# tsolomko/SWCompression

Measured on AMD Instinct MI355X. Metric: decompressed GiB/s, higher is better.
Workload: dtype u8; 1 GPU; 100000 x 64 KiB gzip members (BASELINE configs[1]; 4096 distinct, tiled at distinct addresses); codec=deflate, units_per_gpu=100000, unit_bytes=65536, compressed_bytes_per_gpu=2122936095, decompressed_bytes_per_gpu=6553600000, parallelism=1 x independent shards (weak scaling)

## Files before the change

__graft_entry__.py:

```python
import os
import subprocess
import sys

ROOT = os.path.dirname(os.path.abspath(__file__))
if ROOT not in sys.path:
    sys.path.insert(0, ROOT)


def build():
    from swcompression_amd import build as _b
    _b.build(force=True)
    import swcompression_amd
    from swcompression_amd import _lib
    _lib.load()
    subprocess.run(["make", "-s", "-C", os.path.join(ROOT, "oracle")], check=True)
    sys.path.insert(0, os.path.join(ROOT, "tests"))
    import _emu
    _emu.build(force=True)
    import _emu_bgzf
    _emu_bgzf.build(force=True)


def smoke():
    import torch
    assert torch.cuda.is_available(), "smoke() needs the MI355X"
    sys.path.insert(0, os.path.join(ROOT, "tests"))
    import _oracle as O
    import swcompression_amd as swc
    from swcompression_amd import corpus
    from swcompression_amd.batch import DeviceBatch
    assert swc.device_available(), "libswc_hip.so found no gfx950 device"
    plains = [corpus.p_text(65536, 900 + i) for i in range(96)] + [corpus.p_mix(20000, 5), b"", corpus.p_rand(3000, 1)]
    units = [corpus.deflate_raw(p) for p in plains]
    b = DeviceBatch("deflate", units, [max(len(p), 1) for p in plains], device="cuda:0")
    from swcompression_amd import _lib
    lib = _lib.load()
    expected = [O.deflate(u) for u in units]
    b.launch(sync=True)
    r = b.results()
    for i, (p, (st, out, cons)) in enumerate(zip(plains, expected)):
        assert (st, out) == (0, p)
        assert int(r["status"][i]) == 0 and int(r["out_len"][i]) == len(p) and int(r["in_consumed"][i]) == cons
        assert b.output(i, len(p)) == p, "HIP output differs from the oracle on unit %d" % i
# ... 9 lines not shown
```

include/swc_hip.h:

```cpp
#ifndef SWC_HIP_H
#define SWC_HIP_H

#include <stddef.h>
#include <stdint.h>
#include "swc_status.h"

#ifdef __cplusplus
extern "C" {
#endif

typedef enum swc_codec {
    SWC_CODEC_DEFLATE = 1,
    SWC_CODEC_LZ4_BLOCK = 2,
    SWC_CODEC_LZMA2 = 3,
    SWC_CODEC_LZMA = 4,
    SWC_CODEC_BZIP2_BLOCK = 5,
    SWC_CODEC_DELTA = 6,
    SWC_CODEC_LZ4_COMPRESS = 7,
    SWC_CODEC_DEFLATE_COMPRESS = 8,
    SWC_CODEC_DEFLATE_COMPRESS_DYNAMIC = 9
} swc_codec;

typedef struct swc_job {
    const uint8_t* in;
// ... 2 lines not shown
    uint64_t out_cap;
    uint64_t out_len;
    uint64_t in_consumed;
    int32_t status;
    int32_t aux;
    const uint8_t* dict;
    uint64_t dict_len;
} swc_job;

typedef struct swc_batch_opts {
    int32_t device;
    void* stream;
    int32_t synchronize;
    int32_t reserved;
} swc_batch_opts;

int swc_batch_decompress(int codec, swc_job* jobs, size_t n, const swc_batch_opts* opts);

size_t swc_batch_workspace_bytes(int codec, size_t n_jobs, uint64_t max_out_cap);
int swc_batch_decompress_ws(int codec, swc_job* jobs, size_t n, void* workspace, size_t workspace_bytes,
                            const swc_batch_opts* opts);

int swc_batch_crc32(const swc_job* jobs, size_t n, uint32_t* crcs, const swc_batch_opts* opts);

typedef enum swc_checksum {
    SWC_SUM_CRC32 = 1,
    SWC_SUM_ADLER32 = 2,
    SWC_SUM_CRC64 = 3,
    SWC_SUM_BZIP2_CRC32 = 4,
    SWC_SUM_XXH32 = 5
} swc_checksum;
int swc_batch_checksum(int kind, const swc_job* jobs, size_t n, uint64_t* sums, const swc_batch_opts* opts);

int swc_deflate_decompress(const uint8_t* in, size_t in_len, uint8_t** out, size_t* out_len, size_t* in_consumed);

int swc_bzip2_decompress(const uint8_t* in, size_t in_len, uint8_t** out, size_t* out_len, size_t* in_consumed);
int swc_bzip2_multi_decompress(const uint8_t* in, size_t in_len, uint8_t** out, size_t* out_len, size_t** sizes, size_t* n_streams);

int swc_lzma_decompress(const uint8_t* in, size_t in_len, int lc, int lp, int pb, int64_t dict_size,
                        int64_t uncompressed_size, uint8_t** out, size_t* out_len, size_t* in_consumed);
int swc_lzma_alone_decompress(const uint8_t* in, size_t in_len, uint8_t** out, size_t* out_len);
int swc_lzma2_decompress(const uint8_t* in, size_t in_len, uint8_t dict_byte, uint8_t** out, size_t* out_len, size_t* in_consumed);
int swc_lzma2_decompress_data(const uint8_t* in, size_t in_len, uint8_t** out, size_t* out_len);

int swc_lz4_decompress(const uint8_t* in, size_t in_len, const uint8_t* dict, size_t dict_len, int64_t dict_id,
                       uint8_t** out, size_t* out_len, size_t* in_consumed);
// ... 106 lines not shown
```

swcompression_amd/_lib.py:

```python
import ctypes as C
import os

_HERE = os.path.dirname(os.path.abspath(__file__))
LIB_PATH = os.environ.get("SWC_LIB") or os.path.join(_HERE, "libswc_hip.so")


class SwcJob(C.Structure):
    _fields_ = [("in_", C.c_void_p), ("in_len", C.c_uint64), ("out", C.c_void_p), ("out_cap", C.c_uint64),
                ("out_len", C.c_uint64), ("in_consumed", C.c_uint64), ("status", C.c_int32), ("aux", C.c_int32),
                ("dict", C.c_void_p), ("dict_len", C.c_uint64)]


class SwcGzipExtraField(C.Structure):
    _fields_ = [("si1", C.c_uint8), ("si2", C.c_uint8), ("bytes", C.c_void_p), ("len", C.c_size_t)]


class SwcBatchOpts(C.Structure):
    _fields_ = [("device", C.c_int32), ("stream", C.c_void_p), ("synchronize", C.c_int32), ("reserved", C.c_int32)]


_lib = None


def load():
# ... 11 lines not shown
        raise ImportError("libswc_hip.so is missing and could not be built: the MI355X engine is required")
    lib = C.CDLL(LIB_PATH)
    u8pp = C.POINTER(C.POINTER(C.c_uint8))
    szp = C.POINTER(C.c_size_t)
    szpp = C.POINTER(szp)
    I = C.c_int

    def sig(name, res, *args):
        f = getattr(lib, name)
        f.restype = res
        f.argtypes = list(args)

    sig("swc_free", None, C.c_void_p)
    sig("swc_trim", I)
    sig("swc_device_available", I)
    sig("swc_version", C.c_char_p)
    sig("swc_set_tuning", I, C.c_char_p, I)
    sig("swc_last_phase_ms", I, C.POINTER(C.c_float), I)
    sig("swc_batch_decompress", I, I, C.c_void_p, C.c_size_t, C.POINTER(SwcBatchOpts))
    sig("swc_batch_crc32", I, C.c_void_p, C.c_size_t, C.c_void_p, C.POINTER(SwcBatchOpts))
    sig("swc_batch_checksum", I, I, C.c_void_p, C.c_size_t, C.c_void_p, C.POINTER(SwcBatchOpts))
    sig("swc_batch_workspace_bytes", C.c_size_t, I, C.c_size_t, C.c_uint64)
    sig("swc_batch_decompress_ws", I, I, C.c_void_p, C.c_size_t, C.c_void_p, C.c_size_t, C.POINTER(SwcBatchOpts))
    for n in ("swc_deflate_decompress", "swc_bzip2_decompress"):
        sig(n, I, C.c_char_p, C.c_size_t, u8pp, szp, szp)
    for n in ("swc_gzip_unarchive", "swc_zlib_unarchive", "swc_xz_unarchive", "swc_lzma_alone_decompress", "swc_lzma2_decompress_data"):
        sig(n, I, C.c_char_p, C.c_size_t, u8pp, szp)
    for n in ("swc_gzip_multi_unarchive", "swc_xz_split_unarchive", "swc_bzip2_multi_decompress"):
        sig(n, I, C.c_char_p, C.c_size_t, u8pp, szp, szpp, szp)
    sig("swc_lzma_decompress", I, C.c_char_p, C.c_size_t, I, I, I, C.c_int64, C.c_int64, u8pp, szp, szp)
    sig("swc_lzma2_decompress", I, C.c_char_p, C.c_size_t, C.c_uint8, u8pp, szp, szp)
    sig("swc_lz4_decompress", I, C.c_char_p, C.c_size_t, C.c_char_p, C.c_size_t, C.c_int64, u8pp, szp, szp)
    sig("swc_lz4_multi_decompress", I, C.c_char_p, C.c_size_t, C.c_char_p, C.c_size_t, C.c_int64, u8pp, szp, szpp, szp)
    sig("swc_deflate_compress", I, C.c_char_p, C.c_size_t, u8pp, szp)
    sig("swc_bzip2_compress", I, C.c_char_p, C.c_size_t, I, u8pp, szp)
    sig("swc_zlib_archive", I, C.c_char_p, C.c_size_t, u8pp, szp)
    sig("swc_deflate_compress_dynamic", I, C.c_char_p, C.c_size_t, u8pp, szp)
    sig("swc_zlib_archive_dynamic", I, C.c_char_p, C.c_size_t, u8pp, szp)
    for n in ("swc_gzip_archive", "swc_gzip_archive_dynamic"):
        sig(n, I, C.c_char_p, C.c_size_t, C.c_char_p, C.c_size_t, C.c_char_p, C.c_size_t, I, I, I, I, C.c_int64,
            C.c_void_p, C.c_size_t, u8pp, szp)
    sig("swc_bgzf_bound", C.c_size_t, C.c_size_t, C.c_size_t)
    sig("swc_bgzf_workspace_bytes", C.c_size_t, C.c_size_t, C.c_size_t)
    sig("swc_batch_bgzf_archive", I, C.c_void_p, C.c_uint64, C.c_uint64, I, C.c_void_p, C.c_uint64, C.c_void_p, C.c_void_p,
        C.c_void_p, C.c_size_t, C.POINTER(SwcBatchOpts))
    sig("swc_bgzf_archive", I, C.c_char_p, C.c_size_t, C.c_size_t, I, u8pp, szp, szpp, szp)
# ... 22 lines not shown
```

swcompression_amd/batch.py:

```python
import ctypes as C

import numpy as np

from . import _lib

CODECS = {"deflate": 1, "lz4_block": 2, "lzma2": 3, "lzma": 4, "bzip2_block": 5, "delta": 6, "lz4_compress": 7, "deflate_compress": 8,
          "deflate_compress_dynamic": 9}

JOB_DTYPE = np.dtype([("in", "<u8"), ("in_len", "<u8"), ("out", "<u8"), ("out_cap", "<u8"), ("out_len", "<u8"),
                      ("in_consumed", "<u8"), ("status", "<i4"), ("aux", "<i4"), ("dict", "<u8"), ("dict_len", "<u8")])
assert JOB_DTYPE.itemsize == C.sizeof(_lib.SwcJob) == 72


def _align(x, a=16):
    return (x + a - 1) // a * a


class DeviceBatch:

    def __init__(self, codec, units, caps, aux=None, extra=None, dict_values=None, tile=1, device="cuda:0", replicate_inputs=True,
                 select=None):
        import torch
        self.torch = torch
        self.lib = _lib.load()
# ... 31 lines not shown
        self.d_out = torch.empty(out_total + 16, dtype=torch.uint8, device=self.device)
        jobs = np.zeros(self.n, dtype=JOB_DTYPE)
        jobs["in"] = self.d_in.data_ptr() + ((t_idx - np.uint64(t0)) * np.uint64(in_round) if replicate_inputs else 0) + in_off[k_idx]
        jobs["in_len"] = lens[k_idx]
        jobs["out"] = self.d_out.data_ptr() + out_off
        jobs["out_cap"] = caps[k_idx]
        jobs["status"] = 902
        if aux is not None:
            jobs["aux"] = np.array(aux, dtype=np.int32)[k_idx]
        if extra is not None:
            jobs["dict_len"] = np.array(extra, dtype=np.uint64)[k_idx]
        if dict_values is not None:
            jobs["dict"] = np.array(dict_values, dtype=np.uint64)[k_idx]
        self._out_off = out_off.astype(np.int64)
        self.unit_index = k_idx
        self.caps = caps[k_idx]
        self.in_lens = lens[k_idx]
        self._jobs_host = jobs
        self.d_jobs = torch.from_numpy(jobs.view(np.uint8).copy()).to(self.device)
        ws = self.lib.swc_batch_workspace_bytes(self.codec, self.n, int(caps.max()) if nd else 0)
        self.d_ws = torch.empty(max(ws, 16), dtype=torch.uint8, device=self.device)
        self.ws_bytes = ws
        self._crc_buf = None
        torch.cuda.synchronize(self.device)

    @property
    def total_in(self):
        return int(self.in_lens.sum())

    def launch(self, sync=False):
        torch = self.torch
        opts = _lib.SwcBatchOpts(self.device.index if self.device.index is not None else -1,
                                 torch.cuda.current_stream(self.device).cuda_stream, 1 if sync else 0, 0)
        st = self.lib.swc_batch_decompress_ws(self.codec, self.d_jobs.data_ptr(), self.n, self.d_ws.data_ptr(),
                                              self.ws_bytes, C.byref(opts))
        if st:
            raise RuntimeError("swc_batch_decompress failed with status %d" % st)

    def crc32(self):
        torch = self.torch
        d = torch.empty(self.n, dtype=torch.int32, device=self.device)
        opts = _lib.SwcBatchOpts(self.device.index if self.device.index is not None else -1,
                                 torch.cuda.current_stream(self.device).cuda_stream, 1, 0)
        st = self.lib.swc_batch_crc32(self.d_jobs.data_ptr(), self.n, d.data_ptr(), C.byref(opts))
        if st:
            raise RuntimeError("swc_batch_crc32 failed with status %d" % st)
        return d.cpu().numpy().view(np.uint32)

    def crc32_async(self):
        torch = self.torch
        if self._crc_buf is None:
            self._crc_buf = torch.empty(self.n, dtype=torch.int32, device=self.device)
        opts = _lib.SwcBatchOpts(self.device.index if self.device.index is not None else -1,
                                 torch.cuda.current_stream(self.device).cuda_stream, 0, 0)
        st = self.lib.swc_batch_crc32(self.d_jobs.data_ptr(), self.n, self._crc_buf.data_ptr(), C.byref(opts))
        if st:
            raise RuntimeError("swc_batch_crc32 failed with status %d" % st)

    CHECKSUMS = {"crc32": 1, "adler32": 2, "crc64": 3, "bzip2crc32": 4, "xxh32": 5}

    def checksum(self, kind):
        torch = self.torch
        d = torch.empty(self.n, dtype=torch.int64, device=self.device)
        opts = _lib.SwcBatchOpts(self.device.index if self.device.index is not None else -1,
                                 torch.cuda.current_stream(self.device).cuda_stream, 1, 0)
        st = self.lib.swc_batch_checksum(self.CHECKSUMS[kind], self.d_jobs.data_ptr(), self.n, d.data_ptr(), C.byref(opts))
        if st:
            raise RuntimeError("swc_batch_checksum failed with status %d" % st)
        return d.cpu().numpy().view(np.uint64)

    def wipe_results(self):
        self.d_out.zero_()
        jobs = self._jobs_host.copy()
        jobs["status"] = 902
        jobs["out_len"] = 0
        jobs["in_consumed"] = 0
        self.d_jobs.copy_(self.torch.from_numpy(jobs.view(np.uint8)).to(self.device))
        if self._crc_buf is not None:
            self._crc_buf.zero_()

    def results(self):
        self.torch.cuda.synchronize(self.device)
        return self.d_jobs.cpu().numpy().view(JOB_DTYPE)

    def output(self, i, n=None):
        r = self.results() if n is None else None
        ln = int(min(r["out_len"][i], r["out_cap"][i])) if n is None else n
        o = int(self._out_off[i])
        return self.d_out[o:o + ln].cpu().numpy().tobytes()


def bgzf_workspace_bytes(n_bytes, block_size=65280):
    return _lib.load().swc_bgzf_workspace_bytes(int(n_bytes), int(block_size))

# ... 18 lines not shown
```

swcompression_amd/csrc/api.cpp:

```cpp
#include <algorithm>
#include <atomic>
#include <map>
#include <chrono>
#include <functional>
#include <stdio.h>
#include <stdlib.h>
#include <mutex>
#include <thread>
#include <system_error>
#include <vector>
#include <string.h>
#include "host_util.h"
#include "launch.h"
#include "framing.h"

static_assert(sizeof(swc_job) == sizeof(swc::Job), "swc_job and swc::Job must have the same layout");
static_assert(offsetof(swc_job, status) == offsetof(swc::Job, status), "layout");
static_assert(offsetof(swc_job, dict_len) == offsetof(swc::Job, dict_len), "layout");

namespace swc {

static size_t env_mib(const char* name, size_t dflt) {
    const char* v = getenv(name);
    if (!v || !*v) return dflt;
// ... 268 lines not shown
        uint8_t* up = pinned_stage(0, up_bytes);
        if (!up) { up_fallback.resize(up_bytes); up = up_fallback.data(); }
        for (const Staged& st : staged) if (st.len) memcpy(up + st.off, st.p, st.len);
        Job* jobs = reinterpret_cast<Job*>(up + in_bytes);
        for (size_t k = 0; k < m; k++) {
            const HostUnit& u = units[pending[k]];
            if (u.dict && u.dict_len) memcpy(up + dict_off[k], u.dict, u.dict_len);
            Job& j = jobs[k];
            j.in = d_in + in_off[k];
            j.in_len = u.in_len;
            j.out = d_out + out_off[k];
            j.out_cap = cap[pending[k]];
            j.out_len = 0;
            j.in_consumed = 0;
            j.status = SWC_E_DEVICE;
            j.aux = u.aux;
            j.dict = u.dict ? d_in + dict_off[k] : reinterpret_cast<const uint8_t*>((uintptr_t)u.dict_value);
            j.dict_len = u.dict ? u.dict_len : u.extra;
        }
        if (!ws_off.empty()) memcpy(up + in_bytes + jobs_bytes, ws_off.data(), ws_off.size() * sizeof(uint64_t));
        tr.mark("stage inputs (pinned)", up_bytes);
        if (hipMemcpyAsync(d_in, up, up_bytes, hipMemcpyHostToDevice, stream) != hipSuccess) return SWC_E_DEVICE;
        const uint64_t* d_off = !ws_off.empty() ? reinterpret_cast<const uint64_t*>(d_jobs + jobs_bytes) : nullptr;
        if (launch_codec(codec, reinterpret_cast<Job*>(d_jobs), m, d_ws.ptr(), ws_bytes, stream, d_off) != hipSuccess) return SWC_E_DEVICE;
        if (sum_kind && launch_checksum(sum_kind, reinterpret_cast<const Job*>(d_jobs), m, reinterpret_cast<uint64_t*>(d_sums), stream) != hipSuccess) return SWC_E_DEVICE;
        stat_add(0, 1);
        stat_add(1, (long long)m);
        std::vector<uint8_t> down_fallback;
        uint8_t* down = pinned_stage(1, down_bytes);
        if (!down) { down_fallback.resize(down_bytes); down = down_fallback.data(); }
        if (hipMemcpyAsync(down, d_jobs, down_bytes, hipMemcpyDeviceToHost, stream) != hipSuccess) return SWC_E_DEVICE;
        tr.mark("issue launch + copies");
        if (hipStreamSynchronize(stream) != hipSuccess) return SWC_E_DEVICE;
        tr.mark("H2D + kernels + D2H", down_bytes);
        const Job* res = reinterpret_cast<const Job*>(down);
        const uint64_t* sums = reinterpret_cast<const uint64_t*>(down + jobs_bytes + off_bytes);
        const uint8_t* outs = down + jobs_bytes + off_bytes + sum_bytes;

        std::vector<size_t> next;
        std::vector<CopyOut> done;
        done.reserve(m);
        for (size_t k = 0; k < m; k++) {
            HostUnit& u = units[pending[k]];
            const Job& j = res[k];
            if (j.status == SWC_E_NEED_WORKSPACE && !want_ws) {
                next.push_back(pending[k]);
                continue;
            }
            if (j.status == SWC_E_NEED_WORKSPACE && per_job_ws && ws_extra[pending[k]] == 0) {
                ws_extra[pending[k]] = ((u.in_len * 16 + ((size_t)64 << 10)) + 15) & ~(size_t)15;
                next.push_back(pending[k]);
                continue;
            }
            if (j.status == SWC_E_NEED_WORKSPACE && codec == SWC_CODEC_BZIP2_BLOCK && cap[pending[k]] < ((size_t)15 << 20)) {
                cap[pending[k]] = std::min<size_t>(cap[pending[k]] * 4, (size_t)15 << 20);
                next.push_back(pending[k]);
                continue;
            }
            const size_t grow_limit = codec == SWC_CODEC_BZIP2_BLOCK ? (size_t)1 << 30 : (size_t)1 << 34;
            if (j.status == SWC_E_CAPACITY && !u.cap_exact && cap[pending[k]] < grow_limit) {
                size_t want = j.out_len > cap[pending[k]] ? (size_t)j.out_len : cap[pending[k]] * 4;
                cap[pending[k]] = want;
                next.push_back(pending[k]);
                continue;
            }
            u.status = (j.status == SWC_E_NEED_WORKSPACE && codec == SWC_CODEC_BZIP2_BLOCK) ? (int)SWC_E_CAPACITY : j.status;
            u.aux_out = j.aux;
            u.in_consumed = (size_t)j.in_consumed;
            const size_t produced = (size_t)std::min<uint64_t>(j.out_len, j.out_cap);
            u.out_size = produced;
            u.in_dst = u.dst != nullptr && produced <= u.dst_cap;
            if (sum_kind && u.sum_kind == sum_kind) { u.sum = sums[k]; u.sum_valid = true; }
            done.push_back(CopyOut{&u, outs + out_off[k], produced});
        }
        copy_out(done);
        tr.mark("copy out", out_total);
        if (!next.empty() && !want_ws)
            for (size_t k = 0; k < m; k++)
                if (res[k].status == SWC_E_NEED_WORKSPACE) { want_ws = true; break; }
        next.insert(next.end(), deferred.begin(), deferred.end());
        pending.swap(next);
    }
    for (size_t i : pending) units[i].status = SWC_E_CAPACITY;
    return SWC_OK;
}

}

using namespace swc;

extern "C" {

int swc_set_tuning(const char* key, int value) try {
    if (!key) return SWC_E_INVALID_ARGUMENT;
    if (!strcmp(key, "phase_timing") && (value == 0 || value == 1)) { set_phase_timing(value); return SWC_OK; }
// ... 55 lines not shown
void swc_free(void* p) { host_result_free(p); }

size_t swc_batch_workspace_bytes(int codec, size_t n_jobs, uint64_t max_out_cap) {
    (void)max_out_cap;
    switch (codec) {
        case SWC_CODEC_LZMA:
        case SWC_CODEC_LZMA2: return n_jobs * lzma_spill_bytes_per_job();
        case SWC_CODEC_BZIP2_BLOCK: return n_jobs * bzip2_ws_bytes_per_job((size_t)max_out_cap + 64);
        case SWC_CODEC_DEFLATE: return n_jobs * inflate_ws_bytes_per_job(max_out_cap);
        case SWC_CODEC_LZ4_BLOCK: return n_jobs * lz4_ws_bytes_per_job(max_out_cap);
        default: return 0;
    }
}

int swc_batch_decompress_ws(int codec, swc_job* jobs, size_t n, void* workspace, size_t workspace_bytes,
                            const swc_batch_opts* opts) try {
    if (!device_ready()) return SWC_E_DEVICE;
    if (n && !jobs) return SWC_E_INVALID_ARGUMENT;
    if (opts && opts->device >= 0 && hipSetDevice(opts->device) != hipSuccess) return SWC_E_DEVICE;
    hipStream_t stream = opts ? static_cast<hipStream_t>(opts->stream) : nullptr;
    hipError_t e = launch_codec(codec, reinterpret_cast<Job*>(jobs), n, workspace, workspace_bytes, stream);
    if (e == hipErrorInvalidValue) return SWC_E_INVALID_ARGUMENT;
    if (e != hipSuccess) return SWC_E_DEVICE;
    if (opts && opts->synchronize && hipStreamSynchronize(stream) != hipSuccess) return SWC_E_DEVICE;
    return SWC_OK;
} catch (...) {
    return SWC_E_DEVICE;
}

int swc_batch_crc32(const swc_job* jobs, size_t n, uint32_t* crcs, const swc_batch_opts* opts) try {
    if (!device_ready()) return SWC_E_DEVICE;
    if (n && (!jobs || !crcs)) return SWC_E_INVALID_ARGUMENT;
    if (opts && opts->device >= 0 && hipSetDevice(opts->device) != hipSuccess) return SWC_E_DEVICE;
    hipStream_t stream = opts ? static_cast<hipStream_t>(opts->stream) : nullptr;
    if (launch_crc32(reinterpret_cast<const Job*>(jobs), n, crcs, stream) != hipSuccess) return SWC_E_DEVICE;
    if (opts && opts->synchronize && hipStreamSynchronize(stream) != hipSuccess) return SWC_E_DEVICE;
    return SWC_OK;
} catch (...) {
    return SWC_E_DEVICE;
}

int swc_batch_checksum(int kind, const swc_job* jobs, size_t n, uint64_t* sums, const swc_batch_opts* opts) try {
    if (!device_ready()) return SWC_E_DEVICE;
    if (kind < SWC_SUM_CRC32 || kind > SWC_SUM_XXH32 || (n && (!jobs || !sums))) return SWC_E_INVALID_ARGUMENT;
    if (opts && opts->device >= 0 && hipSetDevice(opts->device) != hipSuccess) return SWC_E_DEVICE;
    hipStream_t stream = opts ? static_cast<hipStream_t>(opts->stream) : nullptr;
// ... 40 lines not shown
```

swcompression_amd/csrc/kernels.hip:

```cpp
#include <hip/hip_runtime.h>
#include <cstddef>
#include <mutex>
#include <atomic>
#include <vector>
#include "swc_common.h"
#include "inflate_lane.h"
#include "inflate_sync.h"
#include "lz_resolve.h"
#include "lz_copy.h"
#include "lz4_lane.h"
#include "lz4_wave.h"
#include "lz4_comp.h"
#include "deflate_comp.h"
#include "lzma_wave.h"
#include "bzip2_block.h"
#include "bzip2_team.h"
#include "crc32_group.h"
#include "crc32_wave.h"
#include "checksum_group.h"
#include "delta_group.h"
#include "bgzf_pack.h"
#include "launch.h"

namespace swc {

struct WsMap {
    uint8_t* base;
    size_t stride;
    const uint64_t* off;
    __device__ uint8_t* area(uint32_t g) const { return base ? base + (off ? (size_t)off[g] : (size_t)g * stride) : nullptr; }
    __device__ size_t bytes(uint32_t g) const { return off ? (size_t)(off[g + 1] - off[g]) : stride; }
};

__device__ __forceinline__ uint32_t xcd_job(uint32_t b, uint32_t n) {
    const uint32_t per = n >> 3;
    return b < (per << 3) ? (b & 7u) * per + (b >> 3) : b;
}

constexpr int kOrderClasses = 256;
constexpr size_t kOrderMin = 2048;
__device__ __forceinline__ uint32_t order_class(uint64_t len) {
// ... 62 lines not shown
#define SWC_SYNC_WAVES_PER_SIMD 4
#endif
static thread_local uint64_t* g_prof = nullptr;
void set_profile_buffer(void* p) { g_prof = static_cast<uint64_t*>(p); }
__global__ __launch_bounds__(64, SWC_SYNC_WAVES_PER_SIMD) void swc_inflate_sync_kernel(Job* __restrict__ jobs, uint32_t n, WsMap wm, uint64_t* prof, const uint32_t* __restrict__ order) {
    __shared__ __attribute__((aligned(16))) inflate::SyncLds sync_lds;
    uint32_t g = job_of(order, blockIdx.x, n);
    if (g >= n) return;
    Job job = jobs[g];
    inflate::inflate_sync_job(job, &sync_lds, wm.area(g), wm.bytes(g), (int)threadIdx.x, kWave, prof ? prof + 32 * (size_t)g : nullptr);
    if (threadIdx.x == 0) put_result(jobs, g, job);
}

constexpr int kInflateResolveThreads = 512, kInflateRingLog2 = 16;
constexpr uint32_t kInflateKeep = 32768;
__global__ __launch_bounds__(kInflateResolveThreads) void swc_lz_resolve_kernel(const Job* __restrict__ jobs, uint32_t n, WsMap wm, uint64_t* prof, const uint32_t* __restrict__ order) {
    __shared__ __attribute__((aligned(16))) lzr::Lds<kInflateResolveThreads, kInflateRingLog2> lzr_lds;
    uint32_t g = job_of(order, blockIdx.x, n);
    if (g >= n) return;
    Job job = jobs[g];
    lzr::resolve_job<kInflateResolveThreads, kInflateRingLog2, kInflateKeep>(job, wm.area(g), wm.bytes(g), &lzr_lds, prof ? prof + 32 * (size_t)g + 16 : nullptr);
}

template <typename CFG, int RM = 0>
__device__ __forceinline__ void lz_copy_body(const Job* __restrict__ jobs, uint32_t n, const WsMap& wm, const uint32_t* __restrict__ order) {
    __shared__ __attribute__((aligned(16))) lzc::Lds<CFG::kWin> lds;
    uint32_t g = job_of(order, blockIdx.x, n);
    if (g >= n) return;
    Job job = jobs[g];
    if (job.dict != nullptr) return;
    lzc::copy_job<CFG, RM>(job, wm.area(g), wm.bytes(g), &lds);
}
#ifndef SWC_LZC_WAVES
#define SWC_LZC_WAVES 6
#endif
#ifndef SWC_LZ4_RECORD_MODE
#define SWC_LZ4_RECORD_MODE 2
#endif
#ifndef SWC_LZC4_WAVES
#define SWC_LZC4_WAVES 5
#endif
__global__ __launch_bounds__(64) __attribute__((amdgpu_waves_per_eu(SWC_LZC_WAVES, SWC_LZC_WAVES))) void swc_lz_copy_kernel(const Job* __restrict__ jobs, uint32_t n, WsMap wm, const uint32_t* __restrict__ order) {
    lz_copy_body<lzc::CfgDeflate>(jobs, n, wm, order);
}
__global__ __launch_bounds__(64) __attribute__((amdgpu_waves_per_eu(SWC_LZC4_WAVES, SWC_LZC4_WAVES))) void swc_lz4_copy_kernel(const Job* __restrict__ jobs, uint32_t n, WsMap wm, const uint32_t* __restrict__ order) {
    lz_copy_body<lzc::CfgLz4, SWC_LZ4_RECORD_MODE>(jobs, n, wm, order);
}
static std::atomic<int> g_lz_copier{1};
void set_lz_copier(int v) { g_lz_copier = v; }
constexpr size_t kCopierMin = 2560;
static bool wave_copier(size_t n) {
    const int c = g_lz_copier;
    return c < 0 || (c == 1 && n >= kCopierMin);
}
static void launch_lz_copy(bool lz4, const Job* jobs, size_t n, const WsMap& wm, const uint32_t* order, hipStream_t stream) {
    if (lz4) hipLaunchKernelGGL(swc_lz4_copy_kernel, dim3((unsigned)n), dim3(kWave), 0, stream, jobs, (uint32_t)n, wm, order);
    else hipLaunchKernelGGL(swc_lz_copy_kernel, dim3((unsigned)n), dim3(kWave), 0, stream, jobs, (uint32_t)n, wm, order);
}

constexpr int kMaxPhases = 8;
struct PhaseTimer {
    int on = 0, n = 0;
    bool ok = false, valid = false;
    hipEvent_t ev[kMaxPhases + 1];
    void begin(hipStream_t s) { n = 0; valid = false; mark(s); }
    void mark(hipStream_t s) {
        if (on && ok && n <= kMaxPhases) { (void)hipEventRecord(ev[n], s); n++; valid = n >= 2; }
    }
};
static thread_local PhaseTimer g_pt;
void set_phase_timing(int on) {
    g_pt.on = on;
    if (on && !g_pt.ok) {
        g_pt.ok = true;
        for (auto& e : g_pt.ev) if (hipEventCreate(&e) != hipSuccess) g_pt.ok = false;
    }
}
int last_phase_ms(float* ms, int cap) {
    if (!g_pt.valid || cap < g_pt.n - 1) return 0;
    if (hipEventSynchronize(g_pt.ev[g_pt.n - 1]) != hipSuccess) return 0;
    for (int i = 0; i + 1 < g_pt.n; i++) if (hipEventElapsedTime(&ms[i], g_pt.ev[i], g_pt.ev[i + 1]) != hipSuccess) return 0;
    return g_pt.n - 1;
}
size_t inflate_ws_bytes_per_job(uint64_t cap) { return lzr::ws_bytes_per_job(cap); }

static std::atomic<int> g_deflate_team{1};
void set_deflate_team(int v) { g_deflate_team = v; }
constexpr size_t kTeamMaxStreams = 256, kTeamForceStreams = 4096;

hipError_t launch_inflate(Job* jobs, size_t n, void* ws, size_t ws_bytes, hipStream_t stream, const uint64_t* ws_off) {
    if (n == 0) return hipSuccess;
    size_t stride = ws ? (ws_bytes / n) & ~(size_t)15 : 0;
    if (!ws_off && stride < sizeof(lzr::StreamHeader)) return hipErrorInvalidValue;
    const WsMap wm{(uint8_t*)ws, stride, ws_off};
    const dim3 block(kWave);
    const int team = g_deflate_team;
    if (!g_prof && ((team == 1 && n <= kTeamMaxStreams) || (team < 0 && n <= kTeamForceStreams))) {
        void* scratch = nullptr;
        if (hipMallocAsync(&scratch, inflate_team_scratch_bytes(n), stream) == hipSuccess) {
            g_pt.begin(stream);
            (void)launch_inflate_team(jobs, n, (uint8_t*)ws, stride, ws_off, (uint8_t*)scratch, stream);
            g_pt.mark(stream);
            (void)hipFreeAsync(scratch, stream);
            const bool copier = wave_copier(n);
            if (copier) launch_lz_copy(false, jobs, n, wm, nullptr, stream);
            else hipLaunchKernelGGL(swc_lz_resolve_kernel, dim3((unsigned)n), dim3(kInflateResolveThreads), 0, stream, jobs, (uint32_t)n, wm, g_prof, (const uint32_t*)nullptr);
            g_pt.mark(stream);
            return hipGetLastError();
        }
        (void)hipGetLastError();
    }
    g_pt.begin(stream);
    const uint32_t* order = job_order(jobs, n, stream);
    hipLaunchKernelGGL(swc_inflate_sync_kernel, dim3((unsigned)n), block, 0, stream, jobs, (uint32_t)n, wm, g_prof, order);
    g_pt.mark(stream);
    const bool copier = wave_copier(n);
    if (copier) launch_lz_copy(false, jobs, n, wm, order, stream);
    else hipLaunchKernelGGL(swc_lz_resolve_kernel, dim3((unsigned)n), dim3(kInflateResolveThreads), 0, stream, jobs, (uint32_t)n, wm, g_prof, order);
    g_pt.mark(stream);
    return hipGetLastError();
}

__global__ __launch_bounds__(64) void swc_lz4_lane_kernel(Job* __restrict__ jobs, uint32_t n, int only_dict) {
    uint32_t g = blockIdx.x * kWave + threadIdx.x;
    if (g >= n) return;
    Job job = jobs[g];
    if (only_dict && job.dict == nullptr) return;
    lz4::lz4_block_job(job);
    put_result(jobs, g, job);
}

#ifndef SWC_LZ4_PARSE_WAVES
#define SWC_LZ4_PARSE_WAVES 4
#endif
template <int RM>
__global__ __launch_bounds__(64) __attribute__((amdgpu_waves_per_eu(SWC_LZ4_PARSE_WAVES))) void swc_lz4_parse_kernel(Job* __restrict__ jobs, uint32_t n, WsMap wm, uint64_t* prof, const uint32_t* __restrict__ order) {
    uint32_t g = job_of(order, blockIdx.x, n);
    if (g >= n) return;
    Job job = jobs[g];
    if (job.dict != nullptr) return;
    __shared__ __attribute__((aligned(16))) uint8_t stage[lz4w::kStageLds];
    lz4w::lz4_parse_job<kWave, RM>(job, wm.area(g), wm.bytes(g), (int)threadIdx.x, stage, prof ? prof + 32 * (size_t)g : nullptr);
// ... 209 lines not shown
    }
    const size_t lcap = lo;
    dim3 block(kWave);
    g_pt.begin(stream);
    const int tw = g_bzip2_team_walk;
    const int team = tw == 2 || (tw == 1 && n * lcap >= kTeamMinBytes) ? 1 : 0;
    if (g_bzip2_hot_cxx) hipLaunchKernelGGL(swc_bzip2_block_kernel<true>, dim3((unsigned)n), block, 0, stream, jobs, (uint32_t)n, (uint8_t*)ws, lcap, team);
    else hipLaunchKernelGGL(swc_bzip2_block_kernel<false>, dim3((unsigned)n), block, 0, stream, jobs, (uint32_t)n, (uint8_t*)ws, lcap, team);
    g_pt.mark(stream);
    if (team) {
        hipLaunchKernelGGL(swc_bzip2_team_prep_kernel, dim3(bzip2::kTeams), block, 0, stream, (uint8_t*)ws, lcap, (uint32_t)n);
        hipLaunchKernelGGL(swc_bzip2_team_walk_kernel, dim3(256), dim3(SWC_BZ_TEAM_THREADS), 0, stream, (uint8_t*)ws, lcap, (uint32_t)n);
        g_pt.mark(stream);
        hipLaunchKernelGGL(swc_bzip2_team_finish_kernel, dim3((unsigned)n), block, 0, stream, jobs, (uint32_t)n, (uint8_t*)ws, lcap);
        g_pt.mark(stream);
    }
    hipLaunchKernelGGL(swc_bzip2_expand_kernel, dim3((unsigned)((n + kWave - 1) / kWave)), block, 0, stream, jobs, (uint32_t)n, (uint8_t*)ws, lcap);
    g_pt.mark(stream);
    hipLaunchKernelGGL(swc_bzip2_crc_kernel, dim3((unsigned)n), dim3(256), 0, stream, jobs, (uint32_t)n);
    g_pt.mark(stream);
    return hipGetLastError();
}

constexpr uint64_t kCrcGroupLen = 1u << 20;
__device__ crcw::WaveConsts g_crc_consts;
__global__ __launch_bounds__(256) void swc_crc32_consts_kernel() { crcw::build_consts<256>(&g_crc_consts, (int)threadIdx.x); }

__global__ __launch_bounds__(256) void swc_crc32_kernel(const Job* __restrict__ jobs, uint32_t n, uint32_t* __restrict__ crcs) {
    __shared__ crcw::WaveConsts lds;
    {
        const uint32_t* src = (const uint32_t*)&g_crc_consts;
        uint32_t* dst = (uint32_t*)&lds;
        constexpr int kWords = (int)(offsetof(crcw::WaveConsts, sq) / 4);
        for (int i = (int)threadIdx.x; i < kWords; i += 256) dst[i] = src[i];
    }
    __syncthreads();
    const uint32_t g = blockIdx.x * 4 + (threadIdx.x >> 6);
    if (g >= n) return;
    const uint64_t len = jobs[g].out_len < jobs[g].out_cap ? jobs[g].out_len : jobs[g].out_cap;
    if (len >= kCrcGroupLen) return;
    const uint32_t c = crcw::crc32_wave((gcptr)jobs[g].out, simt::uniform(len), &lds);
    if ((threadIdx.x & 63) == 0) crcs[g] = c;
}

constexpr int kCrcGroupGrid = 2048;
__global__ __launch_bounds__(256) void swc_crc32_group_kernel(const Job* __restrict__ jobs, uint32_t n, uint32_t* __restrict__ crcs) {
    __shared__ crc::Lds<256> lds;
// ... 1 lines not shown
    __shared__ uint32_t nbig;
    const uint32_t per = (n + gridDim.x - 1) / gridDim.x;
    const uint32_t lo = blockIdx.x * per, hi = lo + per < n ? lo + per : n;
    for (uint32_t base = lo; base < hi; base += 256) {
        if (threadIdx.x == 0) nbig = 0;
        __syncthreads();
        const uint32_t g = base + threadIdx.x;
        if (g < hi) {
            const uint64_t len = jobs[g].out_len < jobs[g].out_cap ? jobs[g].out_len : jobs[g].out_cap;
            if (len >= kCrcGroupLen) big[atomicAdd(&nbig, 1u)] = g;
        }
        __syncthreads();
        const uint32_t cnt = nbig;
        for (uint32_t i = 0; i < cnt; i++) {
            const uint32_t j = big[i];
            const uint64_t len = jobs[j].out_len < jobs[j].out_cap ? jobs[j].out_len : jobs[j].out_cap;
            const uint32_t c = crc::crc32_group<256>((gcptr)jobs[j].out, len, &lds, (int)threadIdx.x);
            if (threadIdx.x == 0) crcs[j] = c;
            __syncthreads();
        }
    }
}

hipError_t launch_crc32(const Job* jobs, size_t n, uint32_t* crcs, hipStream_t stream) {
    if (n == 0) return hipSuccess;
    {
        static std::mutex mu;
        static bool built[64] = {};
        int dev = 0;
        if (hipGetDevice(&dev) != hipSuccess || dev < 0 || dev >= 64) return hipErrorInvalidDevice;
        std::lock_guard<std::mutex> lk(mu);
        if (!built[dev]) {
            hipLaunchKernelGGL(swc_crc32_consts_kernel, dim3(1), dim3(256), 0, stream);
            if (hipStreamSynchronize(stream) != hipSuccess) return hipErrorUnknown;
            built[dev] = true;
        }
    }
    hipLaunchKernelGGL(swc_crc32_kernel, dim3((unsigned)((n + 3) / 4)), dim3(256), 0, stream, jobs, (uint32_t)n, crcs);
    hipLaunchKernelGGL(swc_crc32_group_kernel, dim3((unsigned)(n < (size_t)kCrcGroupGrid ? n : (size_t)kCrcGroupGrid)), dim3(256), 0, stream, jobs, (uint32_t)n, crcs);
    return hipGetLastError();
}

__global__ __launch_bounds__(64) void swc_bgzf_setup_kernel(const uint8_t* src, uint64_t len, uint32_t bs, uint64_t n, Job* cj, Job* kj, uint8_t* slots, uint64_t stride) {
    bgzf::setup_jobs<kWave>(blockIdx.x, src, len, bs, n, cj, kj, slots, stride);
}
__global__ __launch_bounds__(64) void swc_bgzf_scan_kernel(const Job* __restrict__ cj, uint64_t n, uint64_t* offs, uint64_t* sizes, uint64_t* total, bgzf::Result* res, uint64_t dst_cap, int eof) {
    bgzf::scan_members<kWave>(cj, n, offs, sizes, total, res, dst_cap, eof != 0);
}
__global__ __launch_bounds__(64) void swc_bgzf_pack_kernel(uint64_t n, const Job* __restrict__ cj, const Job* __restrict__ kj, const uint32_t* __restrict__ crcs,
                                                           const uint64_t* __restrict__ offs, const bgzf::Result* __restrict__ res, uint8_t* dst, int eof) {
    bgzf::pack_wave<kWave>(blockIdx.x, n, cj, kj, crcs, offs, res, dst, eof != 0);
}
hipError_t launch_bgzf_archive(const uint8_t* src, uint64_t len, uint32_t bs, bool dynamic, uint8_t* dst, uint64_t dst_cap, uint64_t* total,
                               uint64_t* sizes, uint8_t* ws, bool eof, hipStream_t stream) {
    const bgzf::Plan p = bgzf::plan(len, bs);
    if (p.n >= 0x7FFFFFFFull) return hipErrorInvalidValue;
    Job* cj = reinterpret_cast<Job*>(ws + p.cjobs);
    Job* kj = reinterpret_cast<Job*>(ws + p.kjobs);
    uint32_t* crcs = reinterpret_cast<uint32_t*>(ws + p.crcs);
    uint64_t* offs = reinterpret_cast<uint64_t*>(ws + p.offs);
    bgzf::Result* res = reinterpret_cast<bgzf::Result*>(ws + p.res);
    const size_t n = (size_t)p.n;
// ... 85 lines not shown
```

swcompression_amd/csrc/launch.h:

```cpp
#ifndef SWC_LAUNCH_H
#define SWC_LAUNCH_H
#include <hip/hip_runtime.h>
#include "swc_common.h"
namespace swc {
hipError_t launch_inflate(Job* jobs, size_t n, void* ws, size_t ws_bytes, hipStream_t stream, const uint64_t* ws_off = nullptr);
size_t inflate_team_scratch_bytes(size_t n);
hipError_t launch_inflate_team(Job* jobs, size_t n, uint8_t* ws, size_t stride, const uint64_t* ws_off, uint8_t* scratch, hipStream_t stream);
size_t inflate_ws_bytes_per_job(uint64_t cap);
hipError_t launch_crc32(const Job* jobs, size_t n, uint32_t* crcs, hipStream_t stream);
hipError_t launch_delta(Job* jobs, size_t n, hipStream_t stream);
hipError_t launch_checksum(int kind, const Job* jobs, size_t n, uint64_t* sums, hipStream_t stream);
void set_profile_buffer(void* p);
void set_phase_timing(int on);
void set_lzma_coder_cache(int on);
void set_lz_copier(int v);
void set_deflate_team(int v);
void set_bzip2_hot_cxx(int v);
void set_bzip2_team_walk(int v);
int last_phase_ms(float* ms, int cap);
hipError_t launch_lz4(Job* jobs, size_t n, void* ws, size_t ws_bytes, hipStream_t stream, const uint64_t* ws_off = nullptr);
size_t lz4_ws_bytes_per_job(uint64_t cap);
hipError_t launch_lz4_compress(Job* jobs, size_t n, hipStream_t stream);
hipError_t launch_deflate_compress(Job* jobs, size_t n, hipStream_t stream);
hipError_t launch_deflate_compress_dynamic(Job* jobs, size_t n, hipStream_t stream);
hipError_t launch_bgzf_archive(const uint8_t* src, uint64_t len, uint32_t bs, bool dynamic, uint8_t* dst, uint64_t dst_cap, uint64_t* total,
                               uint64_t* sizes, uint8_t* ws, bool eof, hipStream_t stream);
hipError_t launch_lzma(bool lzma2, Job* jobs, size_t n, void* spill, hipStream_t stream);
size_t lzma_spill_bytes_per_job();
// ... 5 lines not shown
```

Baseline: 439.4 GiB/s.

## Fuse gzip CRC32 into the deflate LZ copy kernel

Adds a fused path in which the wave-level LZ copy kernel, after writing each member's output, computes that member's CRC32 in the same block. The CRC constants reuse the LDS window, and the output is read with nontemporal loads while it is likely still in cache. This removes the separate CRC32 kernel pass that re-read all decompressed bytes. Members of 1 MiB or more still go to the group CRC kernel. The fused path is taken only when a CRC buffer already exists, and it adds CRC work to the tail of the copy kernel.

After: 451.3 GiB/s (median of 6 runs). 2.7% higher.

```diff
diff --git a/__graft_entry__.py b/__graft_entry__.py
--- a/__graft_entry__.py
+++ b/__graft_entry__.py
@@ -19,6 +19,8 @@
     _emu.build(force=True)
     import _emu_bgzf
     _emu_bgzf.build(force=True)
+    import _emu_crc_tail
+    _emu_crc_tail.build(force=True)
 
 
 def smoke():
diff --git a/include/swc_hip.h b/include/swc_hip.h
--- a/include/swc_hip.h
+++ b/include/swc_hip.h
@@ -48,6 +48,9 @@
                             const swc_batch_opts* opts);
 
 int swc_batch_crc32(const swc_job* jobs, size_t n, uint32_t* crcs, const swc_batch_opts* opts);
+
+int swc_batch_decompress_crc32_ws(int codec, swc_job* jobs, size_t n, void* workspace, size_t workspace_bytes, uint32_t* crcs,
+                                  const swc_batch_opts* opts);
 
 typedef enum swc_checksum {
     SWC_SUM_CRC32 = 1,
diff --git a/swcompression_amd/_lib.py b/swcompression_amd/_lib.py
--- a/swcompression_amd/_lib.py
+++ b/swcompression_amd/_lib.py
@@ -57,6 +57,7 @@
     sig("swc_batch_checksum", I, I, C.c_void_p, C.c_size_t, C.c_void_p, C.POINTER(SwcBatchOpts))
     sig("swc_batch_workspace_bytes", C.c_size_t, I, C.c_size_t, C.c_uint64)
     sig("swc_batch_decompress_ws", I, I, C.c_void_p, C.c_size_t, C.c_void_p, C.c_size_t, C.POINTER(SwcBatchOpts))
+    sig("swc_batch_decompress_crc32_ws", I, I, C.c_void_p, C.c_size_t, C.c_void_p, C.c_size_t, C.c_void_p, C.POINTER(SwcBatchOpts))
     for n in ("swc_deflate_decompress", "swc_bzip2_decompress"):
         sig(n, I, C.c_char_p, C.c_size_t, u8pp, szp, szp)
     for n in ("swc_gzip_unarchive", "swc_zlib_unarchive", "swc_xz_unarchive", "swc_lzma_alone_decompress", "swc_lzma2_decompress_data"):
diff --git a/swcompression_amd/batch.py b/swcompression_amd/batch.py
--- a/swcompression_amd/batch.py
+++ b/swcompression_amd/batch.py
@@ -77,6 +77,7 @@
         self.d_ws = torch.empty(max(ws, 16), dtype=torch.uint8, device=self.device)
         self.ws_bytes = ws
         self._crc_buf = None
+        self._crc_current = False
         torch.cuda.synchronize(self.device)
 
     @property
@@ -87,8 +88,14 @@
         torch = self.torch
         opts = _lib.SwcBatchOpts(self.device.index if self.device.index is not None else -1,
                                  torch.cuda.current_stream(self.device).cuda_stream, 1 if sync else 0, 0)
-        st = self.lib.swc_batch_decompress_ws(self.codec, self.d_jobs.data_ptr(), self.n, self.d_ws.data_ptr(),
-                                              self.ws_bytes, C.byref(opts))
+        self._crc_current = False
+        if self.codec == CODECS["deflate"] and self._crc_buf is not None:
+            st = self.lib.swc_batch_decompress_crc32_ws(self.codec, self.d_jobs.data_ptr(), self.n, self.d_ws.data_ptr(),
+                                                        self.ws_bytes, self._crc_buf.data_ptr(), C.byref(opts))
+            self._crc_current = st == 0
+        else:
+            st = self.lib.swc_batch_decompress_ws(self.codec, self.d_jobs.data_ptr(), self.n, self.d_ws.data_ptr(),
+                                                  self.ws_bytes, C.byref(opts))
         if st:
             raise RuntimeError("swc_batch_decompress failed with status %d" % st)
 
@@ -104,6 +111,8 @@
 
     def crc32_async(self):
         torch = self.torch
+        if self._crc_current:
+            return
         if self._crc_buf is None:
             self._crc_buf = torch.empty(self.n, dtype=torch.int32, device=self.device)
         opts = _lib.SwcBatchOpts(self.device.index if self.device.index is not None else -1,
@@ -125,6 +134,7 @@
         return d.cpu().numpy().view(np.uint64)
 
     def wipe_results(self):
+        self._crc_current = False
         self.d_out.zero_()
         jobs = self._jobs_host.copy()
         jobs["status"] = 902
diff --git a/swcompression_amd/csrc/api.cpp b/swcompression_amd/csrc/api.cpp
--- a/swcompression_amd/csrc/api.cpp
+++ b/swcompression_amd/csrc/api.cpp
@@ -314,8 +314,13 @@
         tr.mark("stage inputs (pinned)", up_bytes);
         if (hipMemcpyAsync(d_in, up, up_bytes, hipMemcpyHostToDevice, stream) != hipSuccess) return SWC_E_DEVICE;
         const uint64_t* d_off = !ws_off.empty() ? reinterpret_cast<const uint64_t*>(d_jobs + jobs_bytes) : nullptr;
-        if (launch_codec(codec, reinterpret_cast<Job*>(d_jobs), m, d_ws.ptr(), ws_bytes, stream, d_off) != hipSuccess) return SWC_E_DEVICE;
-        if (sum_kind && launch_checksum(sum_kind, reinterpret_cast<const Job*>(d_jobs), m, reinterpret_cast<uint64_t*>(d_sums), stream) != hipSuccess) return SWC_E_DEVICE;
+        const bool fused_crc = codec == SWC_CODEC_DEFLATE && sum_kind == SWC_SUM_CRC32;
+        if (fused_crc) {
+            if (launch_inflate(reinterpret_cast<Job*>(d_jobs), m, d_ws.ptr(), ws_bytes, stream, d_off, reinterpret_cast<uint32_t*>(d_sums)) != hipSuccess) return SWC_E_DEVICE;
+        } else {
+            if (launch_codec(codec, reinterpret_cast<Job*>(d_jobs), m, d_ws.ptr(), ws_bytes, stream, d_off) != hipSuccess) return SWC_E_DEVICE;
+            if (sum_kind && launch_checksum(sum_kind, reinterpret_cast<const Job*>(d_jobs), m, reinterpret_cast<uint64_t*>(d_sums), stream) != hipSuccess) return SWC_E_DEVICE;
+        }
         stat_add(0, 1);
         stat_add(1, (long long)m);
         std::vector<uint8_t> down_fallback;
@@ -362,7 +367,7 @@
             const size_t produced = (size_t)std::min<uint64_t>(j.out_len, j.out_cap);
             u.out_size = produced;
             u.in_dst = u.dst != nullptr && produced <= u.dst_cap;
-            if (sum_kind && u.sum_kind == sum_kind) { u.sum = sums[k]; u.sum_valid = true; }
+            if (sum_kind && u.sum_kind == sum_kind) { u.sum = fused_crc ? reinterpret_cast<const uint32_t*>(sums)[k] : sums[k]; u.sum_valid = true; }
             done.push_back(CopyOut{&u, outs + out_off[k], produced});
         }
         copy_out(done);
@@ -464,6 +469,23 @@
     hipError_t e = launch_codec(codec, reinterpret_cast<Job*>(jobs), n, workspace, workspace_bytes, stream);
     if (e == hipErrorInvalidValue) return SWC_E_INVALID_ARGUMENT;
     if (e != hipSuccess) return SWC_E_DEVICE;
+    if (opts && opts->synchronize && hipStreamSynchronize(stream) != hipSuccess) return SWC_E_DEVICE;
+    return SWC_OK;
+} catch (...) {
+    return SWC_E_DEVICE;
+}
+
+int swc_batch_decompress_crc32_ws(int codec, swc_job* jobs, size_t n, void* workspace, size_t workspace_bytes, uint32_t* crcs,
+                                  const swc_batch_opts* opts) try {
+    if (!device_ready()) return SWC_E_DEVICE;
+    if (n && (!jobs || !crcs)) return SWC_E_INVALID_ARGUMENT;
+    if (opts && opts->device >= 0 && hipSetDevice(opts->device) != hipSuccess) return SWC_E_DEVICE;
+    hipStream_t stream = opts ? static_cast<hipStream_t>(opts->stream) : nullptr;
+    hipError_t e = codec == SWC_CODEC_DEFLATE ? launch_inflate(reinterpret_cast<Job*>(jobs), n, workspace, workspace_bytes, stream, nullptr, crcs)
+                                              : launch_codec(codec, reinterpret_cast<Job*>(jobs), n, workspace, workspace_bytes, stream);
+    if (e == hipErrorInvalidValue) return SWC_E_INVALID_ARGUMENT;
+    if (e != hipSuccess) return SWC_E_DEVICE;
+    if (codec != SWC_CODEC_DEFLATE && launch_crc32(reinterpret_cast<const Job*>(jobs), n, crcs, stream) != hipSuccess) return SWC_E_DEVICE;
     if (opts && opts->synchronize && hipStreamSynchronize(stream) != hipSuccess) return SWC_E_DEVICE;
     return SWC_OK;
 } catch (...) {
diff --git a/swcompression_amd/csrc/crc32_tail.h b/swcompression_amd/csrc/crc32_tail.h
--- /dev/null
+++ b/swcompression_amd/csrc/crc32_tail.h
@@ -0,0 +1,166 @@
+#ifndef SWC_CRC32_TAIL_H
+#define SWC_CRC32_TAIL_H
+
+#include "crc32_wave.h"
+
+namespace swc {
+namespace crct {
+
+using crcw::kPiece;
+using crcw::kRow;
+using crcw::kLevels;
+using crcw::q128u;
+
+struct TailConsts {
+    uint32_t tab[2][256];
+    uint32_t tabg[4][256];
+};
+constexpr uint32_t kTailBytes = 6144;
+static_assert(sizeof(TailConsts) == kTailBytes, "the constants of the tail fill the window and no more");
+static_assert(offsetof(crcw::WaveConsts, tabg) == 4096 && offsetof(crcw::WaveConsts, fold) == 8192, "load_consts copies by offset");
+
+#if defined(__HIP_DEVICE_COMPILE__)
+typedef const __attribute__((address_space(4))) uint32_t* kcptr;
+#else
+typedef const uint32_t* kcptr;
+#endif
+
+SWC_D q128u ld_stream(gcptr p) {
+#if defined(__HIP_DEVICE_COMPILE__)
+    typedef uint32_t u32x4 __attribute__((ext_vector_type(4)));
+    typedef u32x4 __attribute__((aligned(1))) u32x4_any;
+    const u32x4 v = __builtin_nontemporal_load((const SWC_AS_GLOBAL u32x4_any*)p);
+    return q128u{v.x, v.y, v.z, v.w};
+#else
+    return *(const q128u*)p;
+#endif
+}
+SWC_D uint32_t ld_stream32(gcptr p) {
+#if defined(__HIP_DEVICE_COMPILE__)
+    return __builtin_nontemporal_load((const SWC_AS_GLOBAL u32_unaligned*)p);
+#else
+    return load_u32(p);
+#endif
+}
+SWC_D uint32_t ld_stream8(gcptr p) {
+#if defined(__HIP_DEVICE_COMPILE__)
+    return __builtin_nontemporal_load(p);
+#else
+    return *p;
+#endif
+}
+
+SWC_D uint32_t step22(const TailConsts* c, uint32_t s, uint32_t data) {
+    const uint32_t w = s ^ data;
+    const uint32_t u = c->tab[1][w & 0xFF] ^ c->tab[0][(w >> 8) & 0xFF] ^ (w >> 16);
+    return c->tab[1][u & 0xFF] ^ c->tab[0][(u >> 8) & 0xFF] ^ (u >> 16);
+}
+SWC_D uint32_t stepg(const TailConsts* c, uint32_t x) {
+    return c->tabg[0][x & 0xFF] ^ c->tabg[1][(x >> 8) & 0xFF] ^ c->tabg[2][(x >> 16) & 0xFF] ^ c->tabg[3][x >> 24];
+}
+SWC_D uint32_t chain(const TailConsts* c, const q128u& u, const q128u& v) {
+    uint32_t z = step22(c, 0, u.x);
+    z = step22(c, z, u.y);
+    z = step22(c, z, u.z);
+    z = step22(c, z, u.w);
+    z = step22(c, z, v.x);
+    z = step22(c, z, v.y);
+    z = step22(c, z, v.z);
+    return step22(c, z, v.w);
+}
+
+SWC_D uint32_t head_word(gcptr out, int64_t r) {
+    uint32_t w = 0;
+    if (r >= 0) w = ld_stream32(out + r);
+    else if (r > -4) for (int b = (int)-r; b < 4; b++) w |= ld_stream8(out + (r + b)) << (8 * b);
+    if (r > -4 && r < 4) w ^= r >= 0 ? 0xFFFFFFFFu >> (8 * r) : 0xFFFFFFFFu << (8 * -r);
+    return w;
+}
+
+SWC_D void load_consts(TailConsts* c, const crcw::WaveConsts* g) {
+    constexpr int N = kWave;
+    const SWC_AS_GLOBAL q128u* src = (const SWC_AS_GLOBAL q128u*)g;
+    q128u* dst = (q128u*)c;
+    SIMT_BEGIN(t, N)
+#pragma unroll
+        for (int i = t; i < (int)(kTailBytes / 16u); i += N) dst[i] = src[i < 128 ? i : i + 128];
+    SIMT_END_WAVE
+}
+
+SWC_D uint32_t crc32_tail(gcptr out, uint32_t len, TailConsts* c, const crcw::WaveConsts* g) {
+    using namespace simt;
+    constexpr int N = kWave;
+    if (len < 4u) {
+        uint32_t s = 0xFFFFFFFFu;
+        for (uint32_t i = 0; i < len; i++) {
+            s ^= ld_stream8(out + i);
+            for (int k = 0; k < 8; k++) s = (s >> 1) ^ ((s & 1u) ? crcw::kPoly : 0u);
+        }
+        return ~s;
+    }
+    load_consts(c, g);
+    const uint32_t pad = (uint32_t)(kRow - (len & (kRow - 1))) & (kRow - 1);
+    const uint32_t rows = (uint32_t)(((uint64_t)len + pad) / kRow);
+    PT<uint32_t, N> x, y;
+    SIMT_BEGIN(t, N)
+        const int ln = t & (N - 1);
+        const uint32_t first = pad != 0 ? 1 : 0;
+        uint32_t s = 0;
+        const int64_t r0 = (int64_t)ln * kPiece - (int64_t)pad;
+        if (pad != 0 && r0 + kPiece > 0) {
+#pragma unroll
+            for (int k = 0; k < kPiece / 4; k++) s = step22(c, s, head_word(out, r0 + 4 * k));
+        }
+        uint32_t acc = s;
+        const int64_t r1 = r0 + (int64_t)first * kRow;
+        gcptr p = out + r1;
+        uint32_t j = first;
+        const uint32_t init = r1 < 4 ? 0xFFFFFFFFu >> (8 * r1) : 0u;
+        bool fresh = true;
+        if (((rows - first) & 1u) != 0u) {
+            q128u a0 = ld_stream(p), a1 = ld_stream(p + 16);
+            a0.x ^= init;
+            fresh = false;
+            acc = stepg(c, acc) ^ chain(c, a0, a1);
+            p += kRow;
+            j++;
+        }
+        const q128u zero = {0, 0, 0, 0};
+        q128u a[4][2] = {{zero, zero}, {zero, zero}, {zero, zero}, {zero, zero}};
+#pragma unroll
+        for (int k = 0; k < 4; k++)
+            if (j + (uint32_t)k < rows) { a[k][0] = ld_stream(p + k * kRow); a[k][1] = ld_stream(p + k * kRow + 16); }
+        if (fresh) a[0][0].x ^= init;
+        while (j < rows) {
+#pragma unroll
+            for (int h = 0; h < 2; h++) {
+                if (j >= rows) break;
+                const q128u v0 = a[2 * h][0], v1 = a[2 * h][1], v2 = a[2 * h + 1][0], v3 = a[2 * h + 1][1];
+                if (j + 4u < rows) {
+                    a[2 * h][0] = ld_stream(p + 4 * kRow); a[2 * h][1] = ld_stream(p + 4 * kRow + 16);
+                    a[2 * h + 1][0] = ld_stream(p + 5 * kRow); a[2 * h + 1][1] = ld_stream(p + 5 * kRow + 16);
+                }
+                const uint32_t sa = chain(c, v0, v1), sb = chain(c, v2, v3);
+                acc = stepg(c, stepg(c, acc) ^ sa) ^ sb;
+                p += 2 * kRow;
+                j += 2;
+            }
+        }
+        x[t] = acc;
+    SIMT_END
+    kcptr fold = (kcptr)&g->fold[0][0];
+    for (int k = 0; k < kLevels; k++) {
+        wave_shift_down(y, x, 1 << k);
+        SIMT_BEGIN(t, N)
+            uint32_t z = 0;
+#pragma unroll
+            for (int b = 0; b < 32; b++) z ^= (x[t] >> b) & 1u ? fold[32 * k + b] : 0u;
+            x[t] = z ^ y[t];
+        SIMT_END
+    }
+    return ~wave_read(x, 0);
+}
+
+}
+}
+#endif
diff --git a/swcompression_amd/csrc/kernels.hip b/swcompression_amd/csrc/kernels.hip
--- a/swcompression_amd/csrc/kernels.hip
+++ b/swcompression_amd/csrc/kernels.hip
@@ -17,6 +17,7 @@
 #include "bzip2_team.h"
 #include "crc32_group.h"
 #include "crc32_wave.h"
+#include "crc32_tail.h"
 #include "checksum_group.h"
 #include "delta_group.h"
 #include "bgzf_pack.h"
@@ -125,14 +126,26 @@
     lzr::resolve_job<kInflateResolveThreads, kInflateRingLog2, kInflateKeep>(job, wm.area(g), wm.bytes(g), &lzr_lds, prof ? prof + 32 * (size_t)g + 16 : nullptr);
 }
 
-template <typename CFG, int RM = 0>
-__device__ __forceinline__ void lz_copy_body(const Job* __restrict__ jobs, uint32_t n, const WsMap& wm, const uint32_t* __restrict__ order) {
+constexpr uint64_t kCrcGroupLen = 1u << 20;
+extern __device__ crcw::WaveConsts g_crc_consts;
+template <typename CFG, int RM = 0, bool CRC = false>
+__device__ __forceinline__ void lz_copy_body(const Job* __restrict__ jobs, uint32_t n, const WsMap& wm, const uint32_t* __restrict__ order, uint32_t* __restrict__ crcs = nullptr) {
     __shared__ __attribute__((aligned(16))) lzc::Lds<CFG::kWin> lds;
     uint32_t g = job_of(order, blockIdx.x, n);
     if (g >= n) return;
     Job job = jobs[g];
-    if (job.dict != nullptr) return;
-    lzc::copy_job<CFG, RM>(job, wm.area(g), wm.bytes(g), &lds);
+    if constexpr (!CRC) {
+        if (job.dict != nullptr) return;
+        lzc::copy_job<CFG, RM>(job, wm.area(g), wm.bytes(g), &lds);
+    } else {
+        static_assert(sizeof(crct::TailConsts) <= CFG::kWin, "the constants of the tail go where the window was");
+        if (job.dict == nullptr) lzc::copy_job<CFG, RM>(job, wm.area(g), wm.bytes(g), &lds);
+        const uint64_t len = job.out_len < job.out_cap ? job.out_len : job.out_cap;
+        if (len >= kCrcGroupLen) return;
+        simt::vmem_fence();
+        const uint32_t c = crct::crc32_tail((gcptr)job.out, simt::uniform((uint32_t)len), (crct::TailConsts*)lds.win, &g_crc_consts);
+        if (threadIdx.x == 0) crcs[g] = c;
+    }
 }
 #ifndef SWC_LZC_WAVES
 #define SWC_LZC_WAVES 6
@@ -148,6 +161,9 @@
 }
 __global__ __launch_bounds__(64) __attribute__((amdgpu_waves_per_eu(SWC_LZC4_WAVES, SWC_LZC4_WAVES))) void swc_lz4_copy_kernel(const Job* __restrict__ jobs, uint32_t n, WsMap wm, const uint32_t* __restrict__ order) {
     lz_copy_body<lzc::CfgLz4, SWC_LZ4_RECORD_MODE>(jobs, n, wm, order);
+}
+__global__ __launch_bounds__(64) __attribute__((amdgpu_waves_per_eu(SWC_LZC_WAVES, SWC_LZC_WAVES))) void swc_lz_copy_crc32_kernel(const Job* __restrict__ jobs, uint32_t n, WsMap wm, const uint32_t* __restrict__ order, uint32_t* __restrict__ crcs) {
+    lz_copy_body<lzc::CfgDeflate, 0, true>(jobs, n, wm, order, crcs);
 }
 static std::atomic<int> g_lz_copier{1};
 void set_lz_copier(int v) { g_lz_copier = v; }
@@ -191,8 +207,31 @@
 void set_deflate_team(int v) { g_deflate_team = v; }
 constexpr size_t kTeamMaxStreams = 256, kTeamForceStreams = 4096;
 
-hipError_t launch_inflate(Job* jobs, size_t n, void* ws, size_t ws_bytes, hipStream_t stream, const uint64_t* ws_off) {
-    if (n == 0) return hipSuccess;
+static hipError_t crc32_consts_ready(hipStream_t stream);
+static void launch_crc32_group(const Job* jobs, size_t n, uint32_t* crcs, hipStream_t stream);
+static void launch_inflate_phase2(Job* jobs, size_t n, const WsMap& wm, const uint32_t* order, uint32_t* crcs, hipStream_t stream) {
+    if (wave_copier(n)) {
+        if (crcs) {
+            hipLaunchKernelGGL(swc_lz_copy_crc32_kernel, dim3((unsigned)n), dim3(kWave), 0, stream, jobs, (uint32_t)n, wm, order, crcs);
+            g_pt.mark(stream);
+            launch_crc32_group(jobs, n, crcs, stream);
+            return;
+        }
+        launch_lz_copy(false, jobs, n, wm, order, stream);
+        g_pt.mark(stream);
+        return;
+    }
+    hipLaunchKernelGGL(swc_lz_resolve_kernel, dim3((unsigned)n), dim3(kInflateResolveThreads), 0, stream, jobs, (uint32_t)n, wm, g_prof, order);
+    g_pt.mark(stream);
+    if (crcs) (void)launch_crc32(jobs, n, crcs, stream);
+}
+
+hipError_t launch_inflate(Job* jobs, size_t n, void* ws, size_t ws_bytes, hipStream_t stream, const uint64_t* ws_off, uint32_t* crcs) {
+    if (n == 0) return hipSuccess;
+    if (crcs) {
+        const hipError_t e = crc32_consts_ready(stream);
+        if (e != hipSuccess) return e;
+    }
     size_t stride = ws ? (ws_bytes / n) & ~(size_t)15 : 0;
     if (!ws_off && stride < sizeof(lzr::StreamHeader)) return hipErrorInvalidValue;
     const WsMap wm{(uint8_t*)ws, stride, ws_off};
@@ -205,10 +244,7 @@
             (void)launch_inflate_team(jobs, n, (uint8_t*)ws, stride, ws_off, (uint8_t*)scratch, stream);
             g_pt.mark(stream);
             (void)hipFreeAsync(scratch, stream);
-            const bool copier = wave_copier(n);
-            if (copier) launch_lz_copy(false, jobs, n, wm, nullptr, stream);
-            else hipLaunchKernelGGL(swc_lz_resolve_kernel, dim3((unsigned)n), dim3(kInflateResolveThreads), 0, stream, jobs, (uint32_t)n, wm, g_prof, (const uint32_t*)nullptr);
-            g_pt.mark(stream);
+            launch_inflate_phase2(jobs, n, wm, nullptr, crcs, stream);
             return hipGetLastError();
         }
         (void)hipGetLastError();
@@ -217,10 +253,7 @@
     const uint32_t* order = job_order(jobs, n, stream);
     hipLaunchKernelGGL(swc_inflate_sync_kernel, dim3((unsigned)n), block, 0, stream, jobs, (uint32_t)n, wm, g_prof, order);
     g_pt.mark(stream);
-    const bool copier = wave_copier(n);
-    if (copier) launch_lz_copy(false, jobs, n, wm, order, stream);
-    else hipLaunchKernelGGL(swc_lz_resolve_kernel, dim3((unsigned)n), dim3(kInflateResolveThreads), 0, stream, jobs, (uint32_t)n, wm, g_prof, order);
-    g_pt.mark(stream);
+    launch_inflate_phase2(jobs, n, wm, order, crcs, stream);
     return hipGetLastError();
 }
 
@@ -476,7 +509,6 @@
     return hipGetLastError();
 }
 
-constexpr uint64_t kCrcGroupLen = 1u << 20;
 __device__ crcw::WaveConsts g_crc_consts;
 __global__ __launch_bounds__(256) void swc_crc32_consts_kernel() { crcw::build_consts<256>(&g_crc_consts, (int)threadIdx.x); }
 
@@ -524,22 +556,28 @@
     }
 }
 
+static hipError_t crc32_consts_ready(hipStream_t stream) {
+    static std::mutex mu;
+    static bool built[64] = {};
+    int dev = 0;
+    if (hipGetDevice(&dev) != hipSuccess || dev < 0 || dev >= 64) return hipErrorInvalidDevice;
+    std::lock_guard<std::mutex> lk(mu);
+    if (!built[dev]) {
+        hipLaunchKernelGGL(swc_crc32_consts_kernel, dim3(1), dim3(256), 0, stream);
+        if (hipStreamSynchronize(stream) != hipSuccess) return hipErrorUnknown;
+        built[dev] = true;
+    }
+    return hipSuccess;
+}
+static void launch_crc32_group(const Job* jobs, size_t n, uint32_t* crcs, hipStream_t stream) {
+    hipLaunchKernelGGL(swc_crc32_group_kernel, dim3((unsigned)(n < (size_t)kCrcGroupGrid ? n : (size_t)kCrcGroupGrid)), dim3(256), 0, stream, jobs, (uint32_t)n, crcs);
+}
 hipError_t launch_crc32(const Job* jobs, size_t n, uint32_t* crcs, hipStream_t stream) {
     if (n == 0) return hipSuccess;
-    {
-        static std::mutex mu;
-        static bool built[64] = {};
-        int dev = 0;
-        if (hipGetDevice(&dev) != hipSuccess || dev < 0 || dev >= 64) return hipErrorInvalidDevice;
-        std::lock_guard<std::mutex> lk(mu);
-        if (!built[dev]) {
-            hipLaunchKernelGGL(swc_crc32_consts_kernel, dim3(1), dim3(256), 0, stream);
-            if (hipStreamSynchronize(stream) != hipSuccess) return hipErrorUnknown;
-            built[dev] = true;
-        }
-    }
+    const hipError_t e = crc32_consts_ready(stream);
+    if (e != hipSuccess) return e;
     hipLaunchKernelGGL(swc_crc32_kernel, dim3((unsigned)((n + 3) / 4)), dim3(256), 0, stream, jobs, (uint32_t)n, crcs);
-    hipLaunchKernelGGL(swc_crc32_group_kernel, dim3((unsigned)(n < (size_t)kCrcGroupGrid ? n : (size_t)kCrcGroupGrid)), dim3(256), 0, stream, jobs, (uint32_t)n, crcs);
+    launch_crc32_group(jobs, n, crcs, stream);
     return hipGetLastError();
 }
 
diff --git a/swcompression_amd/csrc/launch.h b/swcompression_amd/csrc/launch.h
--- a/swcompression_amd/csrc/launch.h
+++ b/swcompression_amd/csrc/launch.h
@@ -3,7 +3,7 @@
 #include <hip/hip_runtime.h>
 #include "swc_common.h"
 namespace swc {
-hipError_t launch_inflate(Job* jobs, size_t n, void* ws, size_t ws_bytes, hipStream_t stream, const uint64_t* ws_off = nullptr);
+hipError_t launch_inflate(Job* jobs, size_t n, void* ws, size_t ws_bytes, hipStream_t stream, const uint64_t* ws_off = nullptr, uint32_t* crcs = nullptr);
 size_t inflate_team_scratch_bytes(size_t n);
 hipError_t launch_inflate_team(Job* jobs, size_t n, uint8_t* ws, size_t stride, const uint64_t* ws_off, uint8_t* scratch, hipStream_t stream);
 size_t inflate_ws_bytes_per_job(uint64_t cap);
```
